# silverlight6/Ultrasound_Modeling

Hardware: AMD Instinct MI355X
Metric: segmentation training images/sec at 256x256 (higher is better)
Workload: dtype bf16

## Files before the change

### ultrasound_modeling_amd/csrc/common.h

```cpp
#pragma once
#include <hip/hip_runtime.h>
#include <stdint.h>
#include <stdio.h>
#include <stdlib.h>
#include "../../include/usseg.h"
#include "knobs.h"

typedef unsigned short bf16_t;
typedef __attribute__((ext_vector_type(8))) __bf16 bf16x8_t;
typedef __attribute__((ext_vector_type(4))) float f32x4_t;
typedef __attribute__((ext_vector_type(4))) short s16x4_t;

__device__ __forceinline__ float fdiv_rcp(int d) { return 0.5f * __builtin_amdgcn_rcpf((float)d); }
__device__ __forceinline__ int fdiv(int n, float r) {
  float x;
  asm("v_mul_f32_e32 %0, %1, %2" : "=v"(x) : "v"((float)(2 * n + 1)), "v"(r));
  return (int)x;
}
__device__ __forceinline__ void fdivmod(int n, int d, float r, int& q, int& rem) {
  q = fdiv(n, r);
  rem = n - __mul24(q, d);
}

__device__ __forceinline__ float fdiv_rcp1(int d) { return __builtin_amdgcn_rcpf((float)d); }
// ... 385 lines not shown

struct ConvPass {
  const bf16_t* x; const bf16_t* w; void* y; const float* bias; const bf16_t* res;
  const float* scale;
  int B, H, W, d, Cin, ldx, Nout, ldy, ldr, Nw, Kw, ksize, act;
  float alpha;
  int out_f32, accumulate, flip;
  int one_tap;
  UssegTapMask mask;
};
static inline ConvPass conv_pass(const UssegConvJob& q, int flip) {
  const UssegConvDesc& d = q.desc;
  ConvPass p = {};
  p.x = (const bf16_t*)q.x; p.w = (const bf16_t*)q.wp; p.y = q.y; p.res = (const bf16_t*)q.residual; p.ldr = q.ldr;
  p.B = d.B; p.H = d.H; p.W = d.W; p.d = d.dilation; p.ksize = d.ksize;
  p.Cin = flip ? d.Cout : d.Cin; p.ldx = flip ? d.ldy : d.ldx;
  p.Nout = flip ? d.Cin : d.Cout; p.ldy = flip ? d.ldx : d.ldy;
  p.Nw = roundup(p.Nout, 16); p.Kw = d.ksize * d.ksize * p.Cin;
  p.accumulate = (d.flags & USSEG_ACCUMULATE) ? 1 : 0;
  p.flip = flip;
  if (!flip) {
    p.bias = q.bias; p.scale = q.scale;
    p.act = d.act; p.alpha = d.alpha;
    p.out_f32 = (d.flags & USSEG_OUT_F32) ? 1 : 0;
    p.one_tap = d.ksize == 1 && d.dilation == 1;
  }
  return p;
}

void usseg_set_error(const char* fmt, ...);
#define USSEG_CHECK_ARG(cond, ...)                 \
  do {                                             \
    if (!(cond)) {                                 \
      usseg_set_error(__VA_ARGS__);                \
      return USSEG_ERR_BAD_ARG;                    \
    }                                              \
  } while (0)
int usseg_check_launch(const char* what);
int usseg_lds_opt_in(const void* kernel, int bytes);
struct LnTileArgs {
  const bf16_t *x, *dy;
  bf16_t* dx;
  const float *gamma, *beta;
  const float *sa_s, *sa_dg;
  float sa_mult;
  int32_t sa_cy;
  float* ws;
  int64_t M, HW;
  int32_t C, Cphys, G, ldx, lddy, lddx;
  float eps, alpha;
};
int usseg_try_ln_bwd_tile(const LnTileArgs& a, float* dgamma, float* dbeta, float* dbias, float* caller_ws, hipStream_t s);
int usseg_try_ln_bwd_pair(const LnTileArgs& a, float* const* ga, const LnTileArgs& b, float* const* gb, float* caller_ws, hipStream_t s);
int usseg_prof_start(int kind, hipStream_t s);
void usseg_prof_stop(int kind, int slot, hipStream_t s);

#define USSEG_REDUCE_MAX_BLOCKS 1024
void usseg_launch_reduce_finish(const float* ws, int groups, int nb, int K, int Cp, int C, float scale, float* d0, float* d1, float* d2,
                                hipStream_t s, int overwrite = 0);

int usseg_try_launch_conv_big(const ConvPass* p, int njobs, hipStream_t s);
int usseg_try_launch_conv_halo(const ConvPass* p, int njobs, hipStream_t s);

struct WgHaloGeom {
  const bf16_t* x; const bf16_t* dy; float* out; WgMap map;
  int B, H, W, d, Ma, Nb, ldx, lddy;
  int tconv_cls = -1;
  uint32_t tapmask = 0x1ff;
  UssegTapMask mask = {};
};
static inline WgHaloGeom wgrad_halo_geom(const UssegConvDesc& d, const void* x, const void* dy, float* out, const WgMap& map,
                                         const UssegTapMask& mask = {}) {
  WgHaloGeom g = {(const bf16_t*)x, (const bf16_t*)dy, out, map, d.B, d.H, d.W, d.dilation, d.Cin, d.Cout, d.ldx, d.ldy};
  g.mask = mask;
  return g;
}
int usseg_try_launch_wgrad_halo(const WgHaloGeom* g, int njobs, float* ws, int64_t ws_floats, hipStream_t s);
int conv2d_wgrad_impl(const UssegConvDesc* d, const void* x, const void* dy, float* dw, const UssegWgradDst* dst, float* ws, int64_t ws_floats,
                      const UssegTapMask& mask, usseg_stream_t stream);

float* usseg_defer_reduce_ws(hipStream_t s, float* caller_ws, int64_t need);
void usseg_defer_reduce_ws_n(hipStream_t s, float* caller_ws, const int64_t* need, int n, float** out);
float* usseg_defer_wgrad_ws(hipStream_t s, float* caller_ws, int64_t caller_floats, int64_t* avail);
void usseg_launch_wgrad_finish(const float* ws, int splits, int64_t slab_floats, float* out, const WgMap& map, int Ma, int Nb, hipStream_t s);

int usseg_try_launch_tconv_wgrad_halo(const bf16_t* x, const bf16_t* dy, const WgMap& map, int B, int H, int W, int Cin, int Cout, int ldx,
                                      int lddy, int k, float* ws, int64_t ws_floats, hipStream_t s);

static inline int64_t cdiv64(int64_t a, int64_t b) { return (a + b - 1) / b; }
```

### ultrasound_modeling_amd/csrc/conv_big.hip

```cpp
#include "common.h"

struct BigJob {
  const bf16_t* x;
  const bf16_t* w;
  void* y;
  const float* bias;
  const float* scale;
  const bf16_t* res;
  int32_t H, W, d, Hl, Wl, PH, PW, NV;
  int32_t tiles_x, tiles_per_v, npatches;
  int32_t ldx, ldy, ldr, Cin, nchunks, Nw, Kw, Nout, act;
  float alpha;
  int32_t out_f32, accumulate, flip;
  int32_t gx, gy, npa, nstages;
  uint32_t x_bytes, w_bytes;
  int32_t mask_ch;
  int32_t one_tap;
  uint16_t tapmask[4];
};
struct BigParams {
  BigJob job[4];
};

typedef __attribute__((address_space(3))) void* lds_ptr_t;
#define OOB_OFF 0x80000000u

template <int NT, int NS, int NW = 4>
__global__ __launch_bounds__(64 * NW) void conv_big_kernel(const BigParams P) {
#if defined(__HIP_DEVICE_COMPILE__)
  constexpr int BN = 16 * NT;
  constexpr int W_BYTES = 9 * BN * 64;
  constexpr int NPW = 9 * BN / 16;
  constexpr int W_IT = (NPW + NW - 1) / NW;
  constexpr int A_IT = ((NS * NW == 16 ? 36 : 18) + NW - 1) / NW;
  extern __shared__ __attribute__((aligned(1024))) char lds[];
  const BigJob& p = P.job[blockIdx.z];
  if ((int)blockIdx.x >= p.gx || (int)blockIdx.y >= p.gy) return;

  const int tid = threadIdx.x, lane = tid & 63, wv = __builtin_amdgcn_readfirstlane(tid >> 6);
  const int n0 = blockIdx.y * BN;
  const int HW2 = p.PW + 2, HPP = (p.PH + 2) * HW2, NHP = p.NV * HPP;
  const int a_bytes = p.npa * 1024, stage_bytes = a_bytes + W_BYTES;
  const int dd = p.d * p.d;
  const float r_hpp = fdiv_rcp(HPP), r_hw2 = fdiv_rcp(HW2), r_tpv = fdiv_rcp(p.tiles_per_v), r_tx = fdiv_rcp(p.tiles_x), r_dd = fdiv_rcp(dd),
              r_d = fdiv_rcp(p.d);

  const __amdgpu_buffer_rsrc_t rx = __builtin_amdgcn_make_buffer_rsrc((void*)p.x, 0, p.x_bytes, 0x00020000);
  const __amdgpu_buffer_rsrc_t rw = __builtin_amdgcn_make_buffer_rsrc((void*)p.w, 0, p.w_bytes, 0x00020000);
  const int slot_q = (lane & 3) ^ (((lane >> 4) & 1) << 1);
  uint32_t a_off[A_IT], w_off[W_IT];
#pragma unroll
  for (int it = 0; it < A_IT; ++it) {
    const int hp = 16 * (wv + NW * it) + (lane >> 2);
    uint32_t off = OOB_OFF;
    if (hp < NHP) {
      int pi, rem, hy, hx;
      fdivmod(hp, HPP, r_hpp, pi, rem);
      fdivmod(rem, HW2, r_hw2, hy, hx);
      int gp = blockIdx.x * p.NV + pi;
      if (gp < p.npatches) {
        int v, tt, ty, tx, b, ab, la, lb;
        fdivmod(gp, p.tiles_per_v, r_tpv, v, tt);
        fdivmod(tt, p.tiles_x, r_tx, ty, tx);
        fdivmod(v, dd, r_dd, b, ab);
        fdivmod(ab, p.d, r_d, la, lb);
        int ly = __mul24(ty, p.PH) + hy - 1, lx = __mul24(tx, p.PW) + hx - 1;
        if ((unsigned)ly < (unsigned)p.Hl && (unsigned)lx < (unsigned)p.Wl)
          off = (uint32_t)(__mul24(__mul24(__mul24(b, p.H) + la + __mul24(p.d, ly), p.W) + lb + __mul24(p.d, lx), p.ldx) + slot_q * 8) * 2u;
      }
    }
    a_off[it] = off;
  }
#pragma unroll
  for (int it = 0; it < W_IT; ++it) {
    const int row = 16 * (wv + NW * it) + (lane >> 2);
    uint32_t off = OOB_OFF;
    if (row < 9 * BN) {
      int t = row / BN, n = row - t * BN;
// ... 10 lines not shown
    char* wbuf = abuf + a_bytes;
    const uint32_t cb = ck * 64;
    const bool cok = ck * 32 + cq < p.Cin;
#pragma unroll
    for (int it = 0; it < A_IT; ++it) {
      const int j = wv + NW * it;
      if (j < p.npa) {
        __builtin_amdgcn_raw_ptr_buffer_load_lds(rx, (lds_ptr_t)(abuf + j * 1024), 16, cok ? a_off[it] + cb : OOB_OFF, 0, 0, 0);
      }
    }
#pragma unroll
    for (int it = 0; it < W_IT; ++it) {
      const int j = wv + NW * it;
      if (j < NPW) {
        __builtin_amdgcn_raw_ptr_buffer_load_lds(rw, (lds_ptr_t)(wbuf + j * 1024), 16, cok ? w_off[it] + cb : OOB_OFF, 0, 0, 0);
      }
    }
  };

  issue(0, 0);
  const int pl = lane & 15, qk = lane >> 4;
  const int rows_per_strip = 16 / p.PW, spp = (p.PH * p.PW) >> 4;
  int hb[NS];
  int64_t opix[NS];
  bool ovalid[NS];
#pragma unroll
  for (int a = 0; a < NS; ++a) {
    int s = wv * NS + a;
    int pi, sl, r, c;
    fdivmod(s, spp, fdiv_rcp(spp), pi, sl);
    fdivmod(pl, p.PW, fdiv_rcp(p.PW), r, c);
    int row = sl * rows_per_strip + r;
    hb[a] = pi * HPP + row * HW2 + c;
    int gp = blockIdx.x * p.NV + pi;
    ovalid[a] = gp < p.npatches;
    int gpc = ovalid[a] ? gp : 0;
    int v, tt, ty, tx, b, ab, la, lb;
    fdivmod(gpc, p.tiles_per_v, r_tpv, v, tt);
    fdivmod(tt, p.tiles_x, r_tx, ty, tx);
    fdivmod(v, dd, r_dd, b, ab);
    fdivmod(ab, p.d, r_d, la, lb);
    int iy = la + __mul24(p.d, __mul24(ty, p.PH) + row), ix = lb + __mul24(p.d, __mul24(tx, p.PW) + c);
    opix[a] = (int64_t)(__mul24(__mul24(b, p.H) + iy, p.W) + ix);
  }
  const int w_lane = pl * 64 + ((qk ^ (((pl >> 2) & 1) << 1)) << 4);

  f32x4_t acc[NS][NT];
#pragma unroll
  for (int a = 0; a < NS; ++a)
#pragma unroll
    for (int b = 0; b < NT; ++b) acc[a][b] = (f32x4_t){0.f, 0.f, 0.f, 0.f};

  const bool dbuf = p.nstages == 2;
  for (int ck = 0; ck < p.nchunks; ++ck) {
    asm volatile("s_waitcnt vmcnt(0)" ::: "memory");
    __syncthreads();
    if (dbuf && ck + 1 < p.nchunks) issue(ck + 1, (ck + 1) & 1);
    const char* abuf = lds + (dbuf ? (ck & 1) * stage_bytes : 0);
    const char* wbuf = abuf + a_bytes + w_lane;
    const uint32_t tmask = p.one_tap ? 0x010u : (p.mask_ch ? p.tapmask[(p.flip ? ck * 32 : n0) / p.mask_ch] : 0x1ffu);
#pragma unroll
    for (int t = 0; t < 9; ++t) {
      if (!((tmask >> t) & 1u)) continue;
      const int toff = (t / 3) * HW2 + (t % 3);
      bf16x8_t xf[NS], wf[NT];
#pragma unroll
      for (int a = 0; a < NS; ++a) {
        const int hp = hb[a] + toff;
        xf[a] = *reinterpret_cast<const bf16x8_t*>(abuf + (hp << 6) + ((qk << 4) ^ ((hp & 4) << 3)));
      }
#pragma unroll
      for (int b = 0; b < NT; ++b) wf[b] = *reinterpret_cast<const bf16x8_t*>(wbuf + (t * BN + b * 16) * 64);
#pragma unroll
      for (int a = 0; a < NS; ++a)
#pragma unroll
        for (int b = 0; b < NT; ++b) acc[a][b] = __builtin_amdgcn_mfma_f32_16x16x32_bf16(wf[b], xf[a], acc[a][b], 0, 0, 0);
    }
    if (!dbuf && ck + 1 < p.nchunks) {
      __syncthreads();
      issue(ck + 1, 0);
    }
  }

  const EpiArgs e = {p.scale, p.bias, p.res, p.y, p.ldy, p.ldr, p.Nout, p.act, p.alpha, p.out_f32, p.accumulate};
  const int nbase = n0 + qk * 4;
  EpiConst<NT> ec;
  epi_const_load<NT>(ec, p.bias, nbase, p.Nout);
  conv_epilogue<NS, NT>(e, ec, acc, opix, ovalid, nbase);
#endif
}

template <int NT, int NS, bool RES = false>
__global__ __launch_bounds__(256, 2) void conv_stream_kernel(const BigParams P, const int fast_wait) {
#if defined(__HIP_DEVICE_COMPILE__)
  const BigJob& p = P.job[blockIdx.z];
  constexpr int BN = 16 * NT;
  constexpr int W_BYTES = 9 * BN * 64;
  constexpr int NPW = 9 * BN / 16;
  constexpr int A_IT = NS == 4 ? 6 : 3;
  constexpr int MAXG = 64;
  extern __shared__ __attribute__((aligned(1024))) char lds[];
  __shared__ int s_grp[MAXG][4];

  const int tid = threadIdx.x, lane = tid & 63, wv = __builtin_amdgcn_readfirstlane(tid >> 6);
  const int n0 = blockIdx.y * BN;
  const int HW2 = p.PW + 2, NHP = (p.PH + 2) * HW2;
  const int a_bytes = p.npa * 1024;
  char* const wlds = lds;
  char* const alds = lds + p.nchunks * W_BYTES;
  const int dd = p.d * p.d;
  const float r_nch = fdiv_rcp(p.nchunks);
  const float r_hw2 = fdiv_rcp(HW2), r_tpv = fdiv_rcp(p.tiles_per_v), r_tx = fdiv_rcp(p.tiles_x), r_dd = fdiv_rcp(dd), r_d = fdiv_rcp(p.d);

  const int ngroups = p.npatches;
  const int xcd = blockIdx.x & 7, wj = blockIdx.x >> 3, nj = gridDim.x >> 3;
  const int gpx = (ngroups + 7) >> 3;
  const int g_lo = xcd * gpx + wj;
  int g_hi = (xcd + 1) * gpx;
  if (g_hi > ngroups) g_hi = ngroups;
  int ng = g_lo < g_hi ? (g_hi - g_lo + nj - 1) / nj : 0;
  if (ng > MAXG) ng = MAXG;
  if (ng == 0) return;

  const __amdgpu_buffer_rsrc_t rx = __builtin_amdgcn_make_buffer_rsrc((void*)p.x, 0, p.x_bytes, 0x00020000);
  const __amdgpu_buffer_rsrc_t rw = __builtin_amdgcn_make_buffer_rsrc((void*)p.w, 0, p.w_bytes, 0x00020000);
  const int slot_q = (lane & 3) ^ (((lane >> 4) & 1) << 1);
  const int cq = slot_q * 8;

  for (int j = wv; j < p.nchunks * NPW; j += 4) {
// ... 63 lines not shown
        __builtin_amdgcn_raw_ptr_buffer_load_lds(rx, (lds_ptr_t)(abuf + j * 1024), 16, ok ? org + a_rel[it] : OOB_OFF, 0, 0, 0);
      }
    }
  };

  f32x4_t acc[NS][NT];
  const int total = ng * p.nchunks;
  issue_a(0);
  for (int s = 0; s < total; ++s) {
    const int gl = __builtin_amdgcn_readfirstlane(fdiv(s, r_nch)), ck = s - gl * p.nchunks;
    if (fast_wait && s > 0 && ck == 0) asm volatile("s_waitcnt vmcnt(%0) lgkmcnt(0)\n\ts_barrier" ::"n"(NS * NT) : "memory");
    else asm volatile("s_waitcnt vmcnt(0) lgkmcnt(0)\n\ts_barrier" ::: "memory");
    uint2 rr[RES ? NS : 1][RES ? NT : 1];
    if constexpr (RES) {
      if (ck == p.nchunks - 1) {
        const int ob = s_grp[gl][1];
#pragma unroll
        for (int a = 0; a < NS; ++a)
#pragma unroll
          for (int b = 0; b < NT; ++b) {
            const int n = nbase + b * 16;
            rr[a][b] = *reinterpret_cast<const uint2*>(p.res + (int64_t)(ob + orel[a]) * p.ldr + (n < p.Nout ? n : 0));
          }
      }
    }
    if (s + 1 < total) issue_a(s + 1);
    if (ck == 0) {
#pragma unroll
      for (int a = 0; a < NS; ++a)
#pragma unroll
        for (int b = 0; b < NT; ++b) acc[a][b] = (f32x4_t){0.f, 0.f, 0.f, 0.f};
    }
    const char* abuf = alds + (s & 1) * a_bytes;
    const char* wbuf = wlds + ck * W_BYTES + w_lane;
    auto do_tap = [&](int t) {
      const int toff = (t / 3) * HW2 + (t % 3);
      bf16x8_t xf[NS], wf[NT];
#pragma unroll
      for (int a = 0; a < NS; ++a) {
        const int hp = hb[a] + toff;
        xf[a] = *reinterpret_cast<const bf16x8_t*>(abuf + (hp << 6) + ((qk << 4) ^ ((hp & 4) << 3)));
      }
#pragma unroll
      for (int b = 0; b < NT; ++b) wf[b] = *reinterpret_cast<const bf16x8_t*>(wbuf + (t * BN + b * 16) * 64);
#pragma unroll
      for (int a = 0; a < NS; ++a)
#pragma unroll
        for (int b = 0; b < NT; ++b) acc[a][b] = __builtin_amdgcn_mfma_f32_16x16x32_bf16(wf[b], xf[a], acc[a][b], 0, 0, 0);
    };
    if constexpr (RES || NT == 4) {
#pragma unroll
      for (int t = 0; t < 9; ++t) do_tap(t);
    } else if (p.one_tap) do_tap(4);
    else {
#pragma unroll
      for (int t = 0; t < 9; ++t) do_tap(t);
    }
    if (ck != p.nchunks - 1) continue;
    int64_t opix[NS];
    bool ovalid[NS];
    const int obase = s_grp[gl][1];
#pragma unroll
    for (int a = 0; a < NS; ++a) { opix[a] = obase + orel[a]; ovalid[a] = true; }
    if constexpr (RES) {
      const float alpha = p.alpha;
      const int act = p.act;
#pragma unroll
      for (int a = 0; a < NS; ++a) {
        bf16_t* const yrow = reinterpret_cast<bf16_t*>(p.y) + opix[a] * p.ldy;
#pragma unroll
        for (int b = 0; b < NT; ++b) {
          const int n = nbase + b * 16;
          if (n >= p.Nout) continue;
          const float v0 = apply_act(acc[a][b][0] + ec.bb[b].x, act, alpha) + __uint_as_float(rr[a][b].x << 16);
          const float v1 = apply_act(acc[a][b][1] + ec.bb[b].y, act, alpha) + __uint_as_float(rr[a][b].x & 0xffff0000u);
          const float v2 = apply_act(acc[a][b][2] + ec.bb[b].z, act, alpha) + __uint_as_float(rr[a][b].y << 16);
          const float v3 = apply_act(acc[a][b][3] + ec.bb[b].w, act, alpha) + __uint_as_float(rr[a][b].y & 0xffff0000u);
          uint2 o;
          o.x = pack2bf(v0, v1);
          o.y = pack2bf(v2, v3);
          *reinterpret_cast<uint2*>(yrow + n) = o;
        }
      }
    } else {
      conv_epilogue<NS, NT, true>(e, ec, acc, opix, ovalid, nbase);
    }
  }
#endif
}

static int big_fill_job(BigJob& p, const ConvPass& g, int PX, int any_cin = 0) {
  const int min_cin = knob<K_BIG_MIN_CIN>();
  const int B = g.B, H = g.H, W = g.W, d = g.d, ldx = g.ldx;
  if (d < 1 || H % d || W % d || (g.Cin < min_cin && !any_cin)) return 0;
  const int Hl = H / d, Wl = W / d;
  int PW;
  if (Wl % 16 == 0) PW = 16;
  else if (Wl == 8 || Wl == 4) PW = Wl;
  else return 0;
  int PH = PX / PW;
  if (PH > Hl) PH = Hl;
  if (Hl % PH || (PH * PW) % 16 || PX % (PH * PW)) return 0;
  const int NV = PX / (PH * PW);
  const int NHP = NV * (PH + 2) * (PW + 2);
  if (NHP > (PX == 256 ? 576 : 288)) return 0;
  if ((int64_t)B * H * W * ldx >= (1ll << 30) || (int64_t)g.Nw * g.Kw >= (1ll << 30)) return 0;
  if ((int64_t)B * H * W >= (1ll << 23) || (int64_t)B * d * d * (Hl / PH) * (Wl / PW) >= (1ll << 20)) return 0;
  p = {};
  p.x = g.x; p.w = g.w; p.y = g.y; p.bias = g.bias; p.scale = g.scale; p.res = g.res;
  p.H = H; p.W = W; p.d = d; p.Hl = Hl; p.Wl = Wl; p.PH = PH; p.PW = PW; p.NV = NV;
  p.tiles_x = Wl / PW;
  p.tiles_per_v = (Hl / PH) * p.tiles_x;
  p.npatches = B * d * d * p.tiles_per_v;
  p.ldx = ldx; p.ldy = g.ldy; p.ldr = g.ldr; p.Cin = g.Cin; p.nchunks = (g.Cin + 31) / 32;
  p.Nw = g.Nw; p.Kw = g.Kw; p.Nout = g.Nout; p.act = g.act; p.alpha = g.alpha; p.out_f32 = g.out_f32; p.accumulate = g.accumulate; p.flip = g.flip;
  p.gx = (p.npatches + NV - 1) / NV;
  p.x_bytes = (uint32_t)((int64_t)B * H * W * ldx * 2);
  p.w_bytes = (uint32_t)((int64_t)g.Nw * g.Kw * 2);
  p.npa = (NHP + 15) / 16;
  p.mask_ch = g.mask.group_ch;
  for (int c = 0; c < 4; ++c) p.tapmask[c] = g.mask.mask[c];
  p.one_tap = g.one_tap;
  return 1;
}

static int nt_for(int nout) { return nout <= 16 ? 1 : (nout <= 32 ? 2 : 4); }

template <int NT, int NS, int NW = 4>
static void big_launch_t(const BigParams& P, dim3 grid, size_t dyn, hipStream_t s) {
  if (usseg_lds_opt_in((const void*)conv_big_kernel<NT, NS, NW>, 160 * 1024)) return;
  hipLaunchKernelGGL((conv_big_kernel<NT, NS, NW>), grid, dim3(64 * NW), dyn, s, P);
}

static void big_launch(BigParams& P, int njobs, int nt, int PX, hipStream_t s, int w8 = 0) {
  int gx = 0, gy = 0, npa = 0;
  for (int j = 0; j < njobs; ++j) {
    BigJob& p = P.job[j];
    p.gy = (p.Nout + 16 * nt - 1) / (16 * nt);
    if (p.gx > gx) gx = p.gx;
    if (p.gy > gy) gy = p.gy;
    if (p.npa > npa) npa = p.npa;
  }
  const int stages_env = knob<K_BIG_STAGES>();
  int64_t total_wg = 0;
  for (int j = 0; j < njobs; ++j) total_wg += (int64_t)P.job[j].gx * P.job[j].gy;
  const int nstages = stages_env == 2 ? 2 : (stages_env == 1 ? 1 : (total_wg <= 512 ? 2 : 1));
  for (int j = 0; j < njobs; ++j) { P.job[j].npa = npa; P.job[j].nstages = nstages; }
  const size_t dyn = nstages * ((size_t)npa * 1024 + (size_t)9 * 16 * nt * 64);
  const dim3 grid(gx, gy, njobs);
  const int slot = usseg_prof_start(1, s);
  if (PX == 256 && w8) {
    if (nt == 1) big_launch_t<1, 2, 8>(P, grid, dyn, s);
    else if (nt == 2) big_launch_t<2, 2, 8>(P, grid, dyn, s);
    else big_launch_t<4, 2, 8>(P, grid, dyn, s);
  } else if (PX == 256) {
    if (nt == 1) big_launch_t<1, 4>(P, grid, dyn, s);
    else if (nt == 2) big_launch_t<2, 4>(P, grid, dyn, s);
    else big_launch_t<4, 4>(P, grid, dyn, s);
  } else {
    if (nt == 1) big_launch_t<1, 2>(P, grid, dyn, s);
    else if (nt == 2) big_launch_t<2, 2>(P, grid, dyn, s);
    else big_launch_t<4, 2>(P, grid, dyn, s);
  }
  usseg_prof_stop(1, slot, s);
}

template <int NT, int NS, bool RES = false>
static void stream_launch_t(const BigParams& P, dim3 grid, size_t dyn, int fast_wait, hipStream_t s) {
  if (usseg_lds_opt_in((const void*)conv_stream_kernel<NT, NS, RES>, 158 * 1024)) return;
  hipLaunchKernelGGL((conv_stream_kernel<NT, NS, RES>), grid, dim3(256), dyn, s, P, fast_wait);
}

struct StreamPlan {
  BigJob job;
  int nt, PX, res, fast_wait;
  size_t dyn;
  unsigned wgx, gy;
};
static int stream_plan(const ConvPass& g, StreamPlan& sp) {
  const int mode = knob<K_STREAM>();
  const int px_env = knob<K_STREAM_PX>();
  const int min_steps = knob<K_STREAM_MIN_STEPS>();
  const int wgx_env = knob<K_STREAM_WGX>();
  const int occ_env = knob<K_STREAM_OCC>();
  if (!mode || g.mask.group_ch) return 0;
  const int res_env = knob<K_STREAM_RES>();
  if (g.out_f32 || g.accumulate || g.scale) return 0;
  if (g.res && (!res_env || (g.ldr & 3))) return 0;
  const int nt = nt_for(g.Nout);
  const int nchunks = (g.Cin + 31) / 32;
  const size_t wbytes = (size_t)nchunks * 9 * 16 * nt * 64;
  if (wbytes > 40960) return 0;
  const int gy = (g.Nout + 16 * nt - 1) / (16 * nt);
  BigJob& p = sp.job;
  for (int PX = 256; PX >= 128; PX >>= 1) {
    if (px_env && PX != px_env) continue;
    if (!big_fill_job(p, g, PX, 1)) continue;
    if (p.NV != 1 || p.PW != 16) continue;
    if (g.one_tap && (nt == 4 || g.res)) return 0;
    const size_t dyn = wbytes + 2 * (size_t)p.npa * 1024;
    int occ = (int)((160 * 1024 - 2048) / (dyn + 1024));
    if (occ > 4) occ = 4;
    if (occ_env > 0 && occ_env < occ) occ = occ_env;
    if (occ < 1) continue;
    int wgx = (256 * occ / gy) & ~7;
    if (wgx < 8) wgx = 8;
    if (wgx_env >= 8) wgx = wgx_env & ~7;
    const int gpx = (p.npatches + 7) / 8;
    int per_wg = (gpx + wgx / 8 - 1) / (wgx / 8);
    if (per_wg * nchunks < min_steps && !px_env) continue;
    if (per_wg > 64) { wgx = ((gpx + 63) / 64) * 8; per_wg = 64; }
    sp.fast_wait = g.Nout % (16 * nt) == 0 && !g.res;
    sp.nt = nt; sp.PX = PX; sp.res = g.res != nullptr; sp.dyn = dyn; sp.wgx = (unsigned)wgx; sp.gy = (unsigned)gy;
    return 1;
  }
  return 0;
}
static void stream_launch(const StreamPlan* sp, int n, hipStream_t s) {
  BigParams P;
  for (int j = 0; j < n; ++j) P.job[j] = sp[j].job;
  for (int j = n; j < 4; ++j) P.job[j] = sp[0].job;
  const dim3 grid(sp[0].wgx, sp[0].gy, (unsigned)n);
  const int nt = sp[0].nt, PX = sp[0].PX, fast_wait = sp[0].fast_wait;
  const size_t dyn = sp[0].dyn;
  const int slot = usseg_prof_start(1, s);
  if (sp[0].res) {
    if (PX == 256) {
      if (nt == 1) stream_launch_t<1, 4, true>(P, grid, dyn, fast_wait, s);
      else if (nt == 2) stream_launch_t<2, 4, true>(P, grid, dyn, fast_wait, s);
      else stream_launch_t<4, 4, true>(P, grid, dyn, fast_wait, s);
    } else {
      if (nt == 1) stream_launch_t<1, 2, true>(P, grid, dyn, fast_wait, s);
      else if (nt == 2) stream_launch_t<2, 2, true>(P, grid, dyn, fast_wait, s);
      else stream_launch_t<4, 2, true>(P, grid, dyn, fast_wait, s);
    }
  } else if (PX == 256) {
    if (nt == 1) stream_launch_t<1, 4>(P, grid, dyn, fast_wait, s);
    else if (nt == 2) stream_launch_t<2, 4>(P, grid, dyn, fast_wait, s);
    else stream_launch_t<4, 4>(P, grid, dyn, fast_wait, s);
  } else {
    if (nt == 1) stream_launch_t<1, 2>(P, grid, dyn, fast_wait, s);
    else if (nt == 2) stream_launch_t<2, 2>(P, grid, dyn, fast_wait, s);
    else stream_launch_t<4, 2>(P, grid, dyn, fast_wait, s);
  }
  usseg_prof_stop(1, slot, s);
}
static bool stream_same_plan(const StreamPlan& a, const StreamPlan& b) {
  return a.nt == b.nt && a.PX == b.PX && a.res == b.res && a.fast_wait == b.fast_wait && a.dyn == b.dyn && a.wgx == b.wgx && a.gy == b.gy;
}

int usseg_try_launch_conv_big(const ConvPass* g, int njobs, hipStream_t s) {
  const int mode = knob<K_BIG>();
  const int px_env = knob<K_BIG_PX>();
  const int nt_env = knob<K_BIG_NT>();
  const int min_wg = knob<K_BIG_MIN_WG>();
// ... 62 lines not shown
```

### ultrasound_modeling_amd/csrc/knobs.h

```cpp
#pragma once
#include <stdint.h>
#include <stdlib.h>

#define USSEG_KNOBS(X)                                                                                                                  \
                                                                                                                      \
  X(K_BIG,                "USSEG_BIG",                INT,     1,     ONCE,     "0: conv_big and the streaming conv take no launch")        \
  X(K_BIG_PX,             "USSEG_BIG_PX",             INT,     0,     ONCE,     "conv_big: force the pixel tile (128 / 256; 0: planner)")   \
  X(K_BIG_NT,             "USSEG_BIG_NT",             INT,     0,     ONCE,     "conv_big: force the channel tile (1 / 2 / 4 x 16; 0: planner)") \
  X(K_BIG_MIN_WG,         "USSEG_BIG_MIN_WG",         INT,     128,   ONCE,     "conv_big: smallest launch it takes, in workgroups")        \
  X(K_BIG_WG_TILE,        "USSEG_BIG_WG_TILE",        INT,     512,   ONCE,     "conv_big: narrow the channel tile below this many workgroups") \
  X(K_BIG_MIN_CIN,        "USSEG_BIG_MIN_CIN",        INT,     33,    ONCE,     "conv_big: fewest input channels of a pass it takes")       \
  X(K_BIG_STAGES,         "USSEG_BIG_STAGES",         INT,     0,     ONCE,     "conv_big LDS stages: 0 by launch size, 1 / 2 forced")      \
  X(K_BIG_W8,             "USSEG_BIG_W8",             INT,     1,     PER_CALL, "256-pixel tile on eight waves: 0 never, 1 planner, 2 forced") \
  X(K_BIG_W8_MIN,         "USSEG_BIG_W8_MIN",         INT,     128,   ONCE,     "fewest workgroups left for the eight-wave tile")           \
  X(K_STREAM,             "USSEG_STREAM",             INT,     1,     ONCE,     "0: the streaming conv takes no launch")                    \
  X(K_STREAM_PX,          "USSEG_STREAM_PX",          INT,     0,     ONCE,     "streaming conv: force the pixel tile (128 / 256; 0: planner)") \
  X(K_STREAM_MIN_STEPS,   "USSEG_STREAM_MIN_STEPS",   INT,     1,     PER_CALL, "streaming conv: fewest K steps per workgroup it takes")    \
  X(K_STREAM_WGX,         "USSEG_STREAM_WGX",         INT,     0,     PER_CALL, "streaming conv: force grid.x (>= 8, rounded down to a multiple of 8)") \
  X(K_STREAM_OCC,         "USSEG_STREAM_OCC",         INT,     0,     ONCE,     "streaming conv: cap on workgroups per CU (0: by LDS)")     \
  X(K_STREAM_RES,         "USSEG_STREAM_RES",         INT,     1,     ONCE,     "0: passes with a residual do not stream")                  \
  X(K_STREAM_MULTI,       "USSEG_STREAM_MULTI",       INT,     1,     ONCE,     "0: multi-job launches do not stream")                      \
  X(K_STREAM_MERGE,       "USSEG_STREAM_MERGE",       INT,     1,     PER_CALL, "streaming jobs of one plan in one launch (0: a launch per job)") \
                                                                                                     \
  X(K_NO_HALO,            "USSEG_NO_HALO",            PRESENT, 0,     ONCE,     "the halo-tile conv and weight-gradient kernels take no launch") \
  X(K_NO_PERSIST,         "USSEG_NO_PERSIST",         PRESENT, 0,     ONCE,     "conv_halo: never the persistent variant")                  \
  X(K_PERSIST_OCC,        "USSEG_PERSIST_OCC",        INT,     0,     ONCE,     "persistent conv_halo: workgroups per CU (0: by LDS)")      \
                                                                                                                    \
  X(K_IGEMM_WG_MIN,       "USSEG_IGEMM_WG_MIN",       INT,     256,   ONCE,     "igemm: narrow the channel tile below this many workgroups") \
  X(K_IGEMM_KC,           "USSEG_IGEMM_KC",           INT,     0,     ONCE,     "register-staged igemm: force the K step (4 / 8 chunks; 0: by K length)") \
  X(K_IGEMM_DMA,          "USSEG_IGEMM_DMA",          INT,     1,     ONCE,     "0: never the LDS-DMA igemm")                               \
  X(K_IGEMM_DMA_MIN,      "USSEG_IGEMM_DMA_MIN",      INT,     4,     ONCE,     "LDS-DMA igemm: fewest K chunks it takes")                  \
  X(K_IGEMM_DMA_BATCHED,  "USSEG_IGEMM_DMA_BATCHED",  INT,     1,     ONCE,     "0: batched GEMMs stay on the register-staged igemm")       \
  X(K_IGEMM_XCD,          "USSEG_IGEMM_XCD",          INT,     1,     ONCE,     "XCD-aware item order: 0 off, 1 activation-heavy launches, 2 all") \
  X(K_IGEMM_PERSIST,      "USSEG_IGEMM_PERSIST",      INT,     1,     ONCE,     "0: never the persistent LDS-DMA igemm")                    \
  X(K_IGEMM_STAGES8,      "USSEG_IGEMM_STAGES8",      INT,     4,     ONCE,     "ring depth of sparse long-K 128-channel launches (2: off, 3, 4)") \
  X(K_IGEMM_STAGES8_WG,   "USSEG_IGEMM_STAGES8_WG",   INT,     256,   ONCE,     "largest launch, in workgroups, that gets the deeper ring") \
                                                                                                         \
  X(K_WGRAD_DMA,          "USSEG_WGRAD_DMA",          INT,     1,     ONCE,     "0: never the LDS-DMA per-tap weight gradient / batched TN GEMM") \
  X(K_WGRAD_TM,           "USSEG_WGRAD_TM",           INT,     0,     ONCE,     "per-tap wgrad: force the tile (1: 64x64, 2: 128x128; 0: planner)") \
  X(K_WGD_TARGET,         "USSEG_WGD_TARGET",         INT,     512,   ONCE,     "per-tap wgrad: workgroups the split-K aims for")           \
  X(K_WGD_CAP,            "USSEG_WGD_CAP",            INT,     4,     ONCE,     "per-tap wgrad: slab traffic cap, in multiples of the operand bytes") \
  X(K_WG_QUANT,           "USSEG_WG_QUANT",           INT,     1,     ONCE,     "0: no wave-quantisation search of the split count (both wgrad kernels)") \
  X(K_WGRAD_DEBUG,        "USSEG_WGRAD_DEBUG",        PRESENT, 0,     ONCE,     "print every weight-gradient plan to stderr")               \
  X(K_WGRAD_POW2,         "USSEG_WGRAD_POW2",         INT,     1,     ONCE,     "0: no shift decode of power-of-two grids")                 \
  X(K_WGRAD_XCD,          "USSEG_WGRAD_XCD",          INT,     1,     ONCE,     "0: no XCD-aware item order in the per-tap wgrad")          \
  X(K_WG_TARGET,          "USSEG_WG_TARGET",          INT,     256,   ONCE,     "halo wgrad: workgroups the split-K aims for")              \
  X(K_SLAB_CAP,           "USSEG_SLAB_CAP",           INT,     2,     ONCE,     "halo wgrad: slab traffic cap, in multiples of the operand bytes") \
  X(K_WGHALO_XCD,         "USSEG_WGHALO_XCD",         INT,     1,     ONCE,     "0: no XCD-aware item order in the halo wgrad")             \
  X(K_WGRAD_PF,           "USSEG_WGRAD_PF",           INT,     1,     ONCE,     "0: halo wgrad without the register prefetch")              \
  X(K_WGRAD_8W,           "USSEG_WGRAD_8W",           INT,     1,     ONCE,     "0: the 64x64 halo wgrad tile on four waves, not eight")    \
  X(K_TCONV_HALO,         "USSEG_TCONV_HALO",         INT,     0,     PER_CALL, "1: transposed-conv wgrad as four parity-class halo jobs")  \
                                                                                                                      \
  X(K_CARD_BWD_G,         "USSEG_CARD_BWD_G",         INT,     0,     ONCE,     "fused cardinal backward: force the workgroup pairs (0: one resident wave)") \
  X(K_LN_TILE,            "USSEG_LN_TILE",            INT,     1,     ONCE,     "0: never the tile LayerNorm backward")                     \
  X(K_LN_PAIR,            "USSEG_LN_PAIR",            INT,     1,     ONCE,     "0: never the paired LayerNorm backward launch")            \
  X(K_LN_TILE_MIN,        "USSEG_LN_TILE_MIN",        INT,     32768, ONCE,     "fewest pixels for the tile / paired LayerNorm backward")   \
                                                                                     \
  X(K_FLASH_TILE,         "USSEG_FLASH_TILE",         INT,     -1,    ONCE,     "fused attention tiling 0 / 1 / 2 (-1: by problem size)")   \
  X(K_WINATTN_MFMA,       "USSEG_WINATTN_MFMA",       INT,     1,     ONCE,     "0: window attention without the MFMA kernels")             \
  X(K_LOSS_PPT,           "USSEG_LOSS_PPT",           INT,     4,     ONCE,     "softmax + loss kernel: pixels per thread")

enum Knob {
#define X(id, name, kind, def, life, doc) id,
  USSEG_KNOBS(X)
#undef X
};
enum { KNOB_INT, KNOB_PRESENT, KNOB_ONCE, KNOB_PER_CALL };
struct KnobDef { const char* name; int kind; int64_t def; int life; };
constexpr KnobDef kKnobs[] = {
#define X(id, name, kind, def, life, doc) {name, KNOB_##kind, def, KNOB_##life},
  USSEG_KNOBS(X)
#undef X
};

template <Knob K>
// ... 12 lines not shown
```

### ultrasound_modeling_amd/csrc/wgrad_halo.hip

```cpp
#include "common.h"

struct WgHaloParams {
  const bf16_t* x;
  const bf16_t* dy;
  float* out;
  float* ws;
  int32_t B, H, W, d, Hl, Wl, PH, PW, NV;
  int32_t tiles_x, tiles_per_v, npatches, ngroups, groups_per_block;
  int32_t ldx, lddy, Ma, Nb, ntiles_n;
  int32_t mask_ch;
  uint16_t tapmask[4];
  int32_t xvd, xvH, xvW, xva, xvb;
  int32_t yvd, yvH, yvW, yva, yvb;
};

struct WgHaloMulti {
  WgHaloParams job[4];
  int32_t xcd_remap;
};

template <int WVM, int WM, int WN, bool PF, int NTG, bool MASKED>
__global__ __launch_bounds__(256 * NTG, NTG == 1 ? 2 : 1) void wgrad_halo_kernel(const WgHaloMulti P) {
  constexpr int NTHR = 256 * NTG, TPG = NTG == 1 ? 9 : 5;
  int bx = blockIdx.x, by = blockIdx.y, bz = blockIdx.z;
  if (P.xcd_remap) {
    const int gx = gridDim.x, gy = gridDim.y, gz = gridDim.z, total = gx * gy * gz;
    const int L = bx + gx * (by + gy * bz);
    const int c = L & 7, q = total >> 3, r = total & 7;
    const int item = c * q + (c < r ? c : r) + (L >> 3);
    const int u = __builtin_amdgcn_readfirstlane(fdiv(item, fdiv_rcp(gy)));
    by = item - u * gy;
    bx = __builtin_amdgcn_readfirstlane(fdiv(u, fdiv_rcp(gz)));
    bz = u - bx * gz;
  }
  const WgHaloParams& p = P.job[bz];
  constexpr int MAXHP = 288;
  constexpr int WVN = 4 / WVM;
  constexpr int BMc = 16 * WM * WVM, BNc = 16 * WN * WVN;
  constexpr int XS = BMc + 16, YS = BNc == 16 ? 48 : BNc + 16;
  constexpr int XCH = BMc / 8, YCH = BNc / 8;
  constexpr int X_IT = (MAXHP * XCH + NTHR - 1) / NTHR, Y_IT = (128 * YCH + NTHR - 1) / NTHR;
  __shared__ __attribute__((aligned(16))) bf16_t lds_x[MAXHP * XS];
  __shared__ __attribute__((aligned(16))) bf16_t lds_y[128 * YS];
  constexpr int TB = NTHR / 8;
  __shared__ __attribute__((aligned(16))) int s_tab[TB][8][8];

  const int tid = threadIdx.x, lane = tid & 63, wv = (tid >> 6) & 3, tg = tid >> 8;
  const int t0 = tg * TPG;
  const int HW2 = p.PW + 2, HPP = (p.PH + 2) * HW2, NHP = p.NV * HPP;
  const int rps = 16 / p.PW, spp = (p.PH * p.PW) >> 4;
  const float r_hpp = fdiv_rcp(HPP), r_hw2 = fdiv_rcp(HW2), r_spp = fdiv_rcp(spp), r_pw = fdiv_rcp(p.PW), r_tpv = fdiv_rcp(p.tiles_per_v),
              r_tx = fdiv_rcp(p.tiles_x), r_dd = fdiv_rcp(p.d * p.d), r_d = fdiv_rcp(p.d);
  int mt, nt;
  fdivmod(by, p.ntiles_n, fdiv_rcp(p.ntiles_n), mt, nt);
  const int m0 = mt * BMc, n0 = nt * BNc;

  int x_geo[X_IT];
#pragma unroll
  for (int it = 0; it < X_IT; ++it) {
    int idx = tid + NTHR * it;
    int hp = idx / XCH;
    x_geo[it] = -1;
    if (hp < NHP) {
      int pi, rem, hy, hx;
      fdivmod(hp, HPP, r_hpp, pi, rem);
      fdivmod(rem, HW2, r_hw2, hy, hx);
// ... 118 lines not shown
      const bool ok = (x_geo[it] >= 0) & x_cok & ((unsigned)ly < (unsigned)p.Hl) & ((unsigned)lx < (unsigned)p.Wl);
      rx[it] = *reinterpret_cast<const uint4*>(p.x + (ok ? ex[it].x + x_rel[it] : 0));
      mx |= (ok ? 1u : 0u) << it;
    }
#pragma unroll
    for (int it = 0; it < Y_IT; ++it) {
      const bool ok = (tid + NTHR * it < 128 * YCH) & y_cok & (yval[it] != 0);
      ry[it] = *reinterpret_cast<const uint4*>(p.dy + (ok ? yorg[it] + y_rel[it] : 0));
      my |= (ok ? 1u : 0u) << it;
    }
  };
  const uint32_t tmask = (MASKED && p.mask_ch) ? p.tapmask[n0 / p.mask_ch] : 0x1ffu;
  int toff_t[TPG];
#pragma unroll
  for (int tt = 0; tt < TPG; ++tt) {
    const int t = (t0 + tt) < 9 ? (t0 + tt) : 8;
    toff_t[tt] = __builtin_amdgcn_readfirstlane(((t / 3) * HW2 + (t % 3)) * XS);
  }
  const bool last_ok = __builtin_amdgcn_readfirstlane(t0 + TPG - 1) < 9;
  auto compute = [&]() {
    bf16x8_t af[2][WM], bfr[2][WN];
    auto load_b = [&](int ks, bf16x8_t (&b)[WN]) {
#pragma unroll
      for (int j = 0; j < WN; ++j) b[j] = tr8(lds_y, yb[ks][0] + 16 * j, yb[ks][1] + 16 * j);
    };
    auto load_a = [&](int ks, int tt, bf16x8_t (&a)[WM]) {
#pragma unroll
      for (int i = 0; i < WM; ++i) a[i] = tr8(lds_x, xb[ks][0] + toff_t[tt] + 16 * i, xb[ks][1] + toff_t[tt] + 16 * i);
    };
    load_b(0, bfr[0]);
    load_a(0, 0, af[0]);
#pragma unroll
    for (int st = 0; st < 4 * TPG; ++st) {
      const int ks = st / TPG, tt = st - ks * TPG;
      if (st + 1 < 4 * TPG) {
        const int ks1 = (st + 1) / TPG, tt1 = (st + 1) - ks1 * TPG;
        if (tt1 == 0) load_b(ks1, bfr[ks1 & 1]);
        load_a(ks1, tt1, af[(st + 1) & 1]);
      }
      __builtin_amdgcn_sched_barrier(0);
      const bool skip = (NTG > 1 && tt == TPG - 1 && !last_ok) ||
                        (MASKED && !((tmask >> (t0 + tt)) & 1u));
      if (!skip) {
#pragma unroll
        for (int i = 0; i < WM; ++i)
#pragma unroll
          for (int j = 0; j < WN; ++j)
            acc[tt][i][j] = __builtin_amdgcn_mfma_f32_16x16x32_bf16(bfr[ks & 1][j], af[st & 1][i], acc[tt][i][j], 0, 0, 0);
      }
      __builtin_amdgcn_sched_barrier(0);
    }
  };

  if (!PF) {
    for (int grp = g_begin; grp < g_end; ++grp) {
      const int rel = grp - g_begin;
      if ((rel & (TB - 1)) == 0) fill_batch(grp);
      __syncthreads();
      uint4 rx[X_IT], ry[Y_IT];
      uint32_t mx, my;
      load_xy(s_tab[rel & (TB - 1)], rx, ry, mx, my);
#pragma unroll
      for (int it = 0; it < X_IT; ++it)
        if (x_geo[it] >= 0)
          *reinterpret_cast<uint4*>(&lds_x[((tid + NTHR * it) / XCH) * XS + xq * 8]) = (mx >> it) & 1u ? rx[it] : make_uint4(0, 0, 0, 0);
#pragma unroll
      for (int it = 0; it < Y_IT; ++it)
        if (tid + NTHR * it < 128 * YCH)
          *reinterpret_cast<uint4*>(&lds_y[((tid + NTHR * it) / YCH) * YS + yq * 8]) = (my >> it) & 1u ? ry[it] : make_uint4(0, 0, 0, 0);
      __syncthreads();
      compute();
    }
  } else {
    uint4 rx[X_IT], ry[Y_IT];
    uint32_t mx = 0u, my = 0u;
    if (g_begin < g_end) {
      fill_batch(g_begin);
      __syncthreads();
      load_xy(s_tab[0], rx, ry, mx, my);
    }
    for (int grp = g_begin; grp < g_end; ++grp) {
      const int rel1 = grp + 1 - g_begin;
      int (*nxt)[8] = s_tab[rel1 & (TB - 1)];
#pragma unroll
      for (int it = 0; it < X_IT; ++it)
        if (x_geo[it] >= 0)
          *reinterpret_cast<uint4*>(&lds_x[((tid + NTHR * it) / XCH) * XS + xq * 8]) = (mx >> it) & 1u ? rx[it] : make_uint4(0, 0, 0, 0);
#pragma unroll
      for (int it = 0; it < Y_IT; ++it)
        if (tid + NTHR * it < 128 * YCH)
          *reinterpret_cast<uint4*>(&lds_y[((tid + NTHR * it) / YCH) * YS + yq * 8]) = (my >> it) & 1u ? ry[it] : make_uint4(0, 0, 0, 0);
      const bool more = grp + 1 < g_end;
      if (more && (rel1 & (TB - 1)) == 0) fill_batch(grp + 1);
      __syncthreads();
      if (more) {
        load_xy(nxt, rx, ry, mx, my);
      }
      compute();
      __syncthreads();
    }
  }

  float* dst = p.ws ? p.ws + (int64_t)bx * 9 * p.Ma * p.Nb : p.out;
  const bool vec_ok = (p.Nb & 3) == 0;
#pragma unroll
  for (int tt = 0; tt < TPG; ++tt)
#pragma unroll
    for (int i = 0; i < WM; ++i)
#pragma unroll
      for (int j = 0; j < WN; ++j) {
        const int t = t0 + tt;
        if (NTG > 1 && t >= 9) continue;
        const int m = m0 + wm * 16 * WM + i * 16 + li;
        const int n = n0 + wn * 16 * WN + j * 16 + g * 4;
        if (m >= p.Ma || n >= p.Nb) continue;
        float* q = dst + ((int64_t)t * p.Ma + m) * p.Nb + n;
        if (p.ws && vec_ok && n + 3 < p.Nb) {
          *reinterpret_cast<float4*>(q) = make_float4(acc[tt][i][j][0], acc[tt][i][j][1], acc[tt][i][j][2], acc[tt][i][j][3]);
        } else {
#pragma unroll
          for (int r = 0; r < 4; ++r)
            if (n + r < p.Nb) {
              if (p.ws) q[r] = acc[tt][i][j][r];
              else atomicAdd(q + r, acc[tt][i][j][r]);
            }
        }
      }
}

int usseg_try_launch_wgrad_halo(const WgHaloGeom* gm, int njobs, float* ws, int64_t ws_floats, hipStream_t s) {
  const int disabled = knob<K_NO_HALO>();
  if (disabled || njobs < 1 || njobs > 4) return 0;
  WgHaloMulti P;
  const int Ma = gm[0].Ma, Nb = gm[0].Nb;
  auto shape_of = [](int ma, int nb) { return (ma <= 32 && nb <= 32) ? 1 : (nb <= 16 ? 2 : (nb <= 32 ? 3 : 0)); };
  auto tiles_of = [&](int ma, int nb) {
    const int sh = shape_of(ma, nb), bm = sh == 1 ? 32 : 64, bn = sh == 0 ? 64 : (sh == 2 ? 16 : 32);
    return ((ma + bm - 1) / bm) * ((nb + bn - 1) / bn);
  };
  int64_t slab_max = 0, slab_sum = 0;
  for (int j = 0; j < njobs; ++j) {
    const WgHaloGeom& q = gm[j];
    if (q.B != gm[0].B || q.H != gm[0].H || q.W != gm[0].W) return 0;
    if (shape_of(q.Ma, q.Nb) != shape_of(Ma, Nb) || tiles_of(q.Ma, q.Nb) != tiles_of(Ma, Nb)) return 0;
    if ((q.Ma != Ma || q.Nb != Nb) && (q.mask.group_ch || q.tconv_cls >= 0)) return 0;
    slab_sum += (int64_t)9 * q.Ma * q.Nb;
    if ((int64_t)9 * q.Ma * q.Nb > slab_max) slab_max = (int64_t)9 * q.Ma * q.Nb;
    const int d = q.d;
    if (d < 1 || q.H % d || q.W % d) return 0;
    const int Hl = q.H / d, Wl = q.W / d;
    int PW;
    if (Wl % 16 == 0) PW = 16;
    else if (Wl == 8 || Wl == 4) PW = Wl;
    else return 0;
    int PH = 128 / PW;
    if (PH > Hl) PH = Hl;
    if (Hl % PH || (PH * PW) % 16) return 0;
    const int NV = 128 / (PH * PW);
    if (NV * (PH + 2) * (PW + 2) > 288) return 0;
    WgHaloParams& p = P.job[j];
    p = {};
    p.x = q.x; p.dy = q.dy; p.out = q.out;
    p.B = q.B; p.H = q.H; p.W = q.W; p.d = d; p.Hl = Hl; p.Wl = Wl; p.PH = PH; p.PW = PW; p.NV = NV;
    p.tiles_x = Wl / PW;
    p.tiles_per_v = (Hl / PH) * p.tiles_x;
    p.npatches = q.B * d * d * p.tiles_per_v;
    if (q.tconv_cls >= 0) {
      p.xvd = 2; p.xvH = 2 * q.H; p.xvW = 2 * q.W; p.xva = q.tconv_cls >> 1; p.xvb = q.tconv_cls & 1;
      p.yvd = 1; p.yvH = q.H; p.yvW = q.W; p.yva = p.yvb = 0;
      p.mask_ch = 1 << 30;
      p.tapmask[0] = (uint16_t)q.tapmask;
    } else {
      p.xvd = p.yvd = d; p.xvH = p.yvH = q.H; p.xvW = p.yvW = q.W; p.xva = p.xvb = p.yva = p.yvb = 0;
    }
    p.ngroups = (p.npatches + NV - 1) / NV;
    p.ldx = q.ldx; p.lddy = q.lddy; p.Ma = q.Ma; p.Nb = q.Nb;
    if (p.ngroups != P.job[0].ngroups) return 0;
    if ((int64_t)q.B * p.xvH * p.xvW * q.ldx >= (1ll << 31) || (int64_t)q.B * p.yvH * p.yvW * q.lddy >= (1ll << 31)) return 0;
    if ((int64_t)q.B * p.xvH * p.xvW >= (1ll << 23) || (int64_t)q.B * p.yvH * p.yvW >= (1ll << 23) || p.npatches >= (1 << 20)) return 0;
  }
  if (ws) ws = usseg_defer_wgrad_ws(s, ws, ws_floats, &ws_floats);
  int shape = 0;
  if (Ma <= 32 && Nb <= 32) shape = 1;
  else if (Nb <= 16) shape = 2;
  else if (Nb <= 32) shape = 3;
  const int bm = shape == 1 ? 32 : 64, bn = shape == 0 ? 64 : (shape == 2 ? 16 : 32);
  const int tm = (Ma + bm - 1) / bm;
  const int ntn = (Nb + bn - 1) / bn;
  const int tiles = tm * ntn;
  const int ngroups = P.job[0].ngroups;
  const int64_t slab = slab_max;
  int64_t in_bytes = 0;
  for (int j = 0; j < njobs; ++j) in_bytes += (int64_t)gm[j].B * gm[j].H * gm[j].W * (gm[j].Ma + gm[j].Nb) * 2;
  in_bytes /= njobs;
  const int64_t slab_bytes = slab * 4;
  const int wg_target = knob<K_WG_TARGET>();
  int splits = (wg_target + tiles * njobs - 1) / (tiles * njobs);
  int max_splits = (ngroups + 1) / 2;
  const int slab_cap = knob<K_SLAB_CAP>();
  const int64_t traffic_cap = slab_cap * in_bytes / slab_bytes < 4 ? 4 : slab_cap * in_bytes / slab_bytes;
  if (max_splits > traffic_cap) max_splits = (int)traffic_cap;
  if (!ws) max_splits = (ngroups + 15) / 16;
  else if ((int64_t)max_splits * slab_sum > ws_floats) max_splits = (int)(ws_floats / slab_sum);
  if (splits > max_splits) splits = max_splits;
  if (splits < 1) splits = 1;
  {
    const int quant = knob<K_WG_QUANT>();
    if (quant && max_splits > 1) {
      const int slots = 256 * (shape == 0 ? 1 : 2);
      const int64_t tj = (int64_t)tiles * njobs;
      int best = splits;
      double best_cost = 1e30;
      const int lo = splits / 2 > 1 ? splits / 2 : 1, hi = splits * 2 < max_splits ? splits * 2 : max_splits;
      for (int sp = lo; sp <= hi; ++sp) {
        const int g = (ngroups + sp - 1) / sp;
        const int real = (ngroups + g - 1) / g;
        const double rounds = (double)((tj * real + slots - 1) / slots);
        const double cost = rounds * (g + 3.0) + 0.02 * real;
        if (cost < best_cost) { best_cost = cost; best = sp; }
      }
      splits = best;
    }
  }
  bool mapped = false;
  for (int j = 0; j < njobs; ++j) mapped = mapped || gm[j].map.nblocks;
  const bool use_ws = ws && (splits > 1 || mapped) && (int64_t)splits * slab_sum <= ws_floats;
  if (mapped && !use_ws) return 0;
  const int gpb = (ngroups + splits - 1) / splits;
// ... 74 lines not shown
```

Baseline: 5750.

## Reuse each staged pixel row across its three vertical taps in conv and wgrad

Adds a row-reuse path to the big/streaming conv kernels. Each LDS pixel row is read once and fed to all three ty taps that use it, with all nine weight fragments held in registers, which cuts LDS reads roughly threefold. Adds a similar row-reuse compute path to the halo weight-gradient kernel using transposed LDS reads, and caps occupancy for small-NT non-residual streaming launches to make room for the extra registers. Both paths are on by default through a knob bitmask. The cost is much higher register pressure, which could lower occupancy or cause spills.

```diff
diff --git a/ultrasound_modeling_amd/csrc/common.h b/ultrasound_modeling_amd/csrc/common.h
--- a/ultrasound_modeling_amd/csrc/common.h
+++ b/ultrasound_modeling_amd/csrc/common.h
@@ -461,6 +461,7 @@
 };
 int usseg_try_ln_bwd_tile(const LnTileArgs& a, float* dgamma, float* dbeta, float* dbias, float* caller_ws, hipStream_t s);
 int usseg_try_ln_bwd_pair(const LnTileArgs& a, float* const* ga, const LnTileArgs& b, float* const* gb, float* caller_ws, hipStream_t s);
+int usseg_row_reuse_mask();
 int usseg_prof_start(int kind, hipStream_t s);
 void usseg_prof_stop(int kind, int slot, hipStream_t s);
 
diff --git a/ultrasound_modeling_amd/csrc/conv_big.hip b/ultrasound_modeling_amd/csrc/conv_big.hip
--- a/ultrasound_modeling_amd/csrc/conv_big.hip
+++ b/ultrasound_modeling_amd/csrc/conv_big.hip
@@ -1,3 +1,4 @@
+#include <atomic>
 #include "common.h"
 
 struct BigJob {
@@ -17,13 +18,53 @@
   int32_t mask_ch;
   int32_t one_tap;
   uint16_t tapmask[4];
+  int32_t row_reuse;
 };
 struct BigParams {
   BigJob job[4];
 };
 
+static std::atomic<int> g_row_reuse{-1};
+int usseg_row_reuse_mask() {
+  const int v = g_row_reuse.load(std::memory_order_relaxed);
+  return v >= 0 ? v : (int)knob<K_ROW_REUSE>();
+}
+extern "C" int usseg_set_row_reuse(int32_t mask) {
+  g_row_reuse.store(mask, std::memory_order_relaxed);
+  return USSEG_OK;
+}
+
 typedef __attribute__((address_space(3))) void* lds_ptr_t;
 #define OOB_OFF 0x80000000u
+
+template <int NT, int NS>
+__device__ __forceinline__ void chunk_rows(const char* abuf, const char* wbuf, int hb0, int HW2, int qk, f32x4_t (&acc)[NS][NT]) {
+  constexpr int BN = 16 * NT, NF = 3 * (NS + 2), AHEAD = 2;
+  bf16x8_t wf[9][NT];
+#pragma unroll
+  for (int t = 0; t < 9; ++t)
+#pragma unroll
+    for (int b = 0; b < NT; ++b) wf[t][b] = *reinterpret_cast<const bf16x8_t*>(wbuf + (t * BN + b * 16) * 64);
+  auto xread = [&](int i) {
+    const int hp = hb0 + (i / 3) * HW2 + (i % 3);
+    return *reinterpret_cast<const bf16x8_t*>(abuf + (hp << 6) + ((qk << 4) ^ ((hp & 4) << 3)));
+  };
+  bf16x8_t xf[AHEAD + 1];
+#pragma unroll
+  for (int i = 0; i < AHEAD; ++i) xf[i] = xread(i);
+#pragma unroll
+  for (int i = 0; i < NF; ++i) {
+    if (i + AHEAD < NF) xf[(i + AHEAD) % (AHEAD + 1)] = xread(i + AHEAD);
+    const int R = i / 3, tx = i % 3;
+#pragma unroll
+    for (int ty = 0; ty < 3; ++ty) {
+      const int a = R - ty;
+      if (a < 0 || a >= NS) continue;
+#pragma unroll
+      for (int b = 0; b < NT; ++b) acc[a][b] = __builtin_amdgcn_mfma_f32_16x16x32_bf16(wf[ty * 3 + tx][b], xf[i % (AHEAD + 1)], acc[a][b], 0, 0, 0);
+    }
+  }
+}
 
 template <int NT, int NS, int NW = 4>
 __global__ __launch_bounds__(64 * NW) void conv_big_kernel(const BigParams P) {
@@ -140,6 +181,7 @@
     for (int b = 0; b < NT; ++b) acc[a][b] = (f32x4_t){0.f, 0.f, 0.f, 0.f};
 
   const bool dbuf = p.nstages == 2;
+  const bool rows = NT <= 2 && p.row_reuse >= NS;
   for (int ck = 0; ck < p.nchunks; ++ck) {
     asm volatile("s_waitcnt vmcnt(0)" ::: "memory");
     __syncthreads();
@@ -147,22 +189,25 @@
     const char* abuf = lds + (dbuf ? (ck & 1) * stage_bytes : 0);
     const char* wbuf = abuf + a_bytes + w_lane;
     const uint32_t tmask = p.one_tap ? 0x010u : (p.mask_ch ? p.tapmask[(p.flip ? ck * 32 : n0) / p.mask_ch] : 0x1ffu);
-#pragma unroll
-    for (int t = 0; t < 9; ++t) {
-      if (!((tmask >> t) & 1u)) continue;
-      const int toff = (t / 3) * HW2 + (t % 3);
-      bf16x8_t xf[NS], wf[NT];
-#pragma unroll
-      for (int a = 0; a < NS; ++a) {
-        const int hp = hb[a] + toff;
-        xf[a] = *reinterpret_cast<const bf16x8_t*>(abuf + (hp << 6) + ((qk << 4) ^ ((hp & 4) << 3)));
-      }
-#pragma unroll
-      for (int b = 0; b < NT; ++b) wf[b] = *reinterpret_cast<const bf16x8_t*>(wbuf + (t * BN + b * 16) * 64);
-#pragma unroll
-      for (int a = 0; a < NS; ++a)
-#pragma unroll
-        for (int b = 0; b < NT; ++b) acc[a][b] = __builtin_amdgcn_mfma_f32_16x16x32_bf16(wf[b], xf[a], acc[a][b], 0, 0, 0);
+    if (rows) chunk_rows<NT, NS>(abuf, wbuf, hb[0], HW2, qk, acc);
+    else {
+#pragma unroll
+      for (int t = 0; t < 9; ++t) {
+        if (!((tmask >> t) & 1u)) continue;
+        const int toff = (t / 3) * HW2 + (t % 3);
+        bf16x8_t xf[NS], wf[NT];
+#pragma unroll
+        for (int a = 0; a < NS; ++a) {
+          const int hp = hb[a] + toff;
+          xf[a] = *reinterpret_cast<const bf16x8_t*>(abuf + (hp << 6) + ((qk << 4) ^ ((hp & 4) << 3)));
+        }
+#pragma unroll
+        for (int b = 0; b < NT; ++b) wf[b] = *reinterpret_cast<const bf16x8_t*>(wbuf + (t * BN + b * 16) * 64);
+#pragma unroll
+        for (int a = 0; a < NS; ++a)
+#pragma unroll
+          for (int b = 0; b < NT; ++b) acc[a][b] = __builtin_amdgcn_mfma_f32_16x16x32_bf16(wf[b], xf[a], acc[a][b], 0, 0, 0);
+      }
     }
     if (!dbuf && ck + 1 < p.nchunks) {
       __syncthreads();
@@ -332,6 +377,7 @@
 #pragma unroll
       for (int t = 0; t < 9; ++t) do_tap(t);
     } else if (p.one_tap) do_tap(4);
+    else if (p.row_reuse >= NS) chunk_rows<NT, NS>(abuf, wbuf, hb[0], HW2, qk, acc);
     else {
 #pragma unroll
       for (int t = 0; t < 9; ++t) do_tap(t);
@@ -401,6 +447,7 @@
   p.mask_ch = g.mask.group_ch;
   for (int c = 0; c < 4; ++c) p.tapmask[c] = g.mask.mask[c];
   p.one_tap = g.one_tap;
+  if ((usseg_row_reuse_mask() & 1) && PW == 16 && !p.one_tap && !p.mask_ch) p.row_reuse = PH % 4 == 0 ? 4 : (PH % 2 == 0 ? 2 : 0);
   return 1;
 }
 
@@ -481,6 +528,10 @@
     const size_t dyn = wbytes + 2 * (size_t)p.npa * 1024;
     int occ = (int)((160 * 1024 - 2048) / (dyn + 1024));
     if (occ > 4) occ = 4;
+    if (!g.res && nt <= 2) {
+      const int rocc = PX == 256 ? 2 : (nt == 1 ? 4 : 3);
+      if (occ > rocc) occ = rocc;
+    }
     if (occ_env > 0 && occ_env < occ) occ = occ_env;
     if (occ < 1) continue;
     int wgx = (256 * occ / gy) & ~7;
diff --git a/ultrasound_modeling_amd/csrc/knobs.h b/ultrasound_modeling_amd/csrc/knobs.h
--- a/ultrasound_modeling_amd/csrc/knobs.h
+++ b/ultrasound_modeling_amd/csrc/knobs.h
@@ -21,6 +21,7 @@
   X(K_STREAM_RES,         "USSEG_STREAM_RES",         INT,     1,     ONCE,     "0: passes with a residual do not stream")                  \
   X(K_STREAM_MULTI,       "USSEG_STREAM_MULTI",       INT,     1,     ONCE,     "0: multi-job launches do not stream")                      \
   X(K_STREAM_MERGE,       "USSEG_STREAM_MERGE",       INT,     1,     PER_CALL, "streaming jobs of one plan in one launch (0: a launch per job)") \
+  X(K_ROW_REUSE,          "USSEG_ROW_REUSE",          INT,     3,     ONCE,     "read each staged pixel row once for its three taps: bit 0 conv_big / streaming conv, bit 1 halo wgrad") \
                                                                                                      \
   X(K_NO_HALO,            "USSEG_NO_HALO",            PRESENT, 0,     ONCE,     "the halo-tile conv and weight-gradient kernels take no launch") \
   X(K_NO_PERSIST,         "USSEG_NO_PERSIST",         PRESENT, 0,     ONCE,     "conv_halo: never the persistent variant")                  \
diff --git a/ultrasound_modeling_amd/csrc/wgrad_halo.hip b/ultrasound_modeling_amd/csrc/wgrad_halo.hip
--- a/ultrasound_modeling_amd/csrc/wgrad_halo.hip
+++ b/ultrasound_modeling_amd/csrc/wgrad_halo.hip
@@ -12,6 +12,7 @@
   uint16_t tapmask[4];
   int32_t xvd, xvH, xvW, xva, xvb;
   int32_t yvd, yvH, yvW, yva, yvb;
+  int32_t row_reuse;
 };
 
 struct WgHaloMulti {
@@ -236,6 +237,49 @@
     }
   };
 
+  constexpr bool ROWS = PF && NTG == 1 && !MASKED && WVM == 2 && WM == 1 && WN == 1;
+  auto compute_rows = [&]() {
+   if constexpr (ROWS) {
+    constexpr int RS = 18 * XS;
+    const bf16_t* xbase = lds_x + xb[0][0];
+    auto half = [&](int R, int tx, int i) -> s16x4_t {
+      return __builtin_amdgcn_ds_read_tr16_b64_v4i16((s16x4_t __attribute__((address_space(3)))*)(xbase + R * RS + tx * XS + 16 * i));
+    };
+    s16x4_t hv[10][3][WM];
+    bf16x8_t bfr[2][WN];
+#pragma unroll
+    for (int j = 0; j < WN; ++j) bfr[0][j] = tr8(lds_y, yb[0][0] + 16 * j, yb[0][1] + 16 * j);
+#pragma unroll
+    for (int r = 0; r < 2; ++r)
+#pragma unroll
+      for (int tx = 0; tx < 3; ++tx)
+#pragma unroll
+        for (int i = 0; i < WM; ++i) hv[r][tx][i] = half(r, tx, i);
+#pragma unroll
+    for (int st = 0; st < 36; ++st) {
+      const int ks = st / 9, tt = st - ks * 9, ty = tt / 3, tx = tt - ty * 3;
+      if (tt < 6) {
+#pragma unroll
+        for (int i = 0; i < WM; ++i) hv[2 * ks + 2 + ty][tx][i] = half(2 * ks + 2 + ty, tx, i);
+      } else if (tt == 6 && ks < 3) {
+#pragma unroll
+        for (int j = 0; j < WN; ++j) bfr[(ks + 1) & 1][j] = tr8(lds_y, yb[ks + 1][0] + 16 * j, yb[ks + 1][1] + 16 * j);
+      }
+      __builtin_amdgcn_sched_barrier(0);
+#pragma unroll
+      for (int i = 0; i < WM; ++i) {
+        const s16x4_t lo = hv[2 * ks + ty][tx][i], hi = hv[2 * ks + ty + 1][tx][i];
+        const s16x8_t v = {lo[0], lo[1], lo[2], lo[3], hi[0], hi[1], hi[2], hi[3]};
+#pragma unroll
+        for (int j = 0; j < WN; ++j)
+          acc[tt][i][j] = __builtin_amdgcn_mfma_f32_16x16x32_bf16(bfr[ks & 1][j], __builtin_bit_cast(bf16x8_t, v), acc[tt][i][j], 0, 0, 0);
+      }
+      __builtin_amdgcn_sched_barrier(0);
+    }
+   }
+  };
+  const bool rows = ROWS && p.row_reuse;
+
   if (!PF) {
     for (int grp = g_begin; grp < g_end; ++grp) {
       const int rel = grp - g_begin;
@@ -280,7 +324,8 @@
       if (more) {
         load_xy(nxt, rx, ry, mx, my);
       }
-      compute();
+      if (rows) compute_rows();
+      else compute();
       __syncthreads();
     }
   }
@@ -358,6 +403,7 @@
       p.xvd = p.yvd = d; p.xvH = p.yvH = q.H; p.xvW = p.yvW = q.W; p.xva = p.xvb = p.yva = p.yvb = 0;
     }
     p.ngroups = (p.npatches + NV - 1) / NV;
+    p.row_reuse = (usseg_row_reuse_mask() & 2) && NV == 1 && PW == 16;
     p.ldx = q.ldx; p.lddy = q.lddy; p.Ma = q.Ma; p.Nb = q.Nb;
     if (p.ngroups != P.job[0].ngroups) return 0;
     if ((int64_t)q.B * p.xvH * p.xvW * q.ldx >= (1ll << 31) || (int64_t)q.B * p.yvH * p.yvW * q.lddy >= (1ll << 31)) return 0;
```

After: 5752 (median of 4 runs). Within noise of the previous version (+0.0%).
